# weihaoysgs/ssvio

Hardware: AMD Instinct MI355X
Metric: stereo frames/s (ORB extract + row-band match + triangulate + one local BA per frame) on 1241x376 (higher is better)
Workload: dtype u8 (front-end) + f64 (BA)

## Files before the change

### include/ssx_test_hooks.h

```cpp
#ifndef SSX_TEST_HOOKS_H
#define SSX_TEST_HOOKS_H
#include "ssx.h"

#ifdef __cplusplus
extern "C" {
#endif

SSX_API int32_t ssx_ba_window_selftest(uint32_t seed, int32_t steps);

SSX_API int64_t ssx_debug_kernel_dynamic_lds(const char* kernel);
SSX_API void ssx_debug_set_dense_slabs(int32_t mode);

SSX_API void ssx_debug_set_trial_finish(int32_t mode);

SSX_API double ssx_ba_debug_prepare_seconds(const ssx_ba_problem* prob, int32_t reps);

SSX_API int32_t ssx_ba_debug_upload_format(const ssx_ba_problem* prob);

SSX_API uint64_t ssx_ba_debug_prepare_digest(const ssx_ba_problem* prob, int32_t threads);

typedef struct ssx_orb_plan_info {
  int32_t status, n_buffers;
  uint64_t digest[3];
  uint64_t arena_bytes, buf_off[32], buf_bytes[32];
  int32_t nlevels, out_cap;
  int32_t lvl_rows[8], lvl_cols[8], feat[8], lvl_cell0[9], gauss_tile0[9];
  char error[256];
} ssx_orb_plan_info;
SSX_API ssx_status ssx_orb_debug_plan(int32_t rows, int32_t cols, int32_t images, const ssx_orb_params* prm, int32_t has_mask,
                                      int32_t detect_only, int32_t unchecked, ssx_orb_plan_info* out);


// ... 46 lines not shown
```

### ssvio_amd/csrc/ba.hip

```cpp
#include <algorithm>
#include <atomic>
#include <chrono>
#include <cmath>
#include <limits>
#include <map>
#include <condition_variable>
#include <functional>
#include <mutex>
#include <numeric>
#include <thread>
#include <unordered_map>
#include <vector>

#include <cstring>
#include <rocprim/device/device_radix_sort.hpp>
#include <rocprim/device/device_run_length_encode.hpp>
#include <rocprim/device/device_scan.hpp>

#include "ctx.hpp"
#include "se3.hpp"
#include "../../include/ssx_test_hooks.h"

int ssx_comm_allreduce_f64(void* user, double* buf_dev, size_t count, void* stream);

// ... 11 lines not shown
#ifndef SSX_LIN_VA
#define SSX_LIN_VA 14
#endif
#ifndef SSX_LS_WGS
#define SSX_LS_WGS 3
#endif
constexpr int CH_E = SSX_CHUNK_E;
constexpr int PW = CH_E + 2;
constexpr int CH_L = SSX_CHUNK_L;
constexpr int PL = CH_L + 1;
constexpr int SSX_BA_SMALL_P = 16;
constexpr int UPPER6 = 21;
constexpr int TOUCH_WORDS = (SSX_BA_SMALL_P * (SSX_BA_SMALL_P + 1) / 2 + SSX_BA_SMALL_P + 31) / 32;
constexpr int BSEG_PARTS = 4;
constexpr int BSEG_MIN = 8;
constexpr int MAX_PAIRS = CH_E * (SSX_BA_SMALL_P + 1) / 2 + 8;

template <class T>
struct GPtr {
  T* p;
#if defined(__HIP_DEVICE_COMPILE__)
  using G = __attribute__((address_space(1))) T*;
#else
  using G = T*;
#endif
  __host__ __device__ __forceinline__ GPtr& operator=(T* q) { p = q; return *this; }
  __host__ __device__ __forceinline__ operator G() const { return (G)p; }
  __host__ __device__ __forceinline__ G get() const { return (G)p; }
};
#if defined(__HIP_DEVICE_COMPILE__)
// ... 22 lines not shown
  GPtr<const uint8_t> e_cam;
  GPtr<const uint8_t> e_dup;
  GPtr<const double> e_uv;
  GPtr<const int8_t> blk_pa;
  GPtr<const int8_t> blk_pb;
  GPtr<const int4> ch_desc;
  GPtr<const int4> e_rec;
  GPtr<const int4> l_rec;
  GPtr<const uint16_t> pptr;
  GPtr<uint8_t> pair_a;
  GPtr<uint8_t> pair_b;
  GPtr<int> pair_ptr;
  GPtr<int4> bseg;
  GPtr<int> bseg_ptr;
  int bseg_cap;
  int dev_prep;
  int E_raw;
  GPtr<const int> r_edge_pose;
  GPtr<const int> r_edge_point;
  GPtr<const double> r_edge_uv;
  GPtr<const uint8_t> r_edge_cam;
  GPtr<const uint8_t> r_slot8;
  int no_err;
  int raw_fmt;
  GPtr<const int> lm_compact;
  GPtr<const int> pose_rank;
  GPtr<int> perm;
  GPtr<int> lm_chunk;
  GPtr<double> c2_out;
  Cam K;
// ... 486 lines not shown
{
  if (threadIdx.x == 0 && blockIdx.x == 0) d.scal[SC_LAMBDA] = lambda;
}

constexpr int LIST_MAX_BLK = SSX_BA_SMALL_P * (SSX_BA_SMALL_P + 1) / 2;
__device__ __forceinline__ void k_build_lists_body(const BaDev& d, const int c)
{
  __shared__ uint8_t sEdgeOf[CH_L][SSX_BA_SMALL_P];
  __shared__ int8_t sLead[CH];
  __shared__ int sCnt[2][LIST_MAX_BLK];
  __shared__ int sBp[LIST_MAX_BLK + 1];
  __shared__ int sLen[LIST_MAX_BLK], sK[LIST_MAX_BLK];
  __shared__ uint8_t sSorted[LIST_MAX_BLK];
  __shared__ int sMaxLen, sWaveTot[4], sWaveMax[4];
  __shared__ int sPosR[LIST_MAX_BLK + 1];
  __shared__ int sKr[LIST_MAX_BLK];
  const int t = threadIdx.x, lane = t & 63, wave = t >> 6;
  const int4 cd = d.ch_desc[c];
  const int e0 = cd.x, lm0 = cd.z, nl = cd.w;
  const int nP = d.nP, nBlk = d.nBlk;
  const unsigned long long lt_mask = (1ull << lane) - 1ull;
  if (t < cd.y) {
    const int4 er = d.e_rec[e0 + t];
    sLead[t] = (er.y >= 0 && !(er.w & 2)) ? (int8_t)er.y : (int8_t)-1;
  }
  int4 lr = make_int4(0, 0, 0, 1);
  if (t < nl) lr = d.l_rec[lm0 + t];
  __syncthreads();
  uint32_t mask = 0;
  if (t < nl && !lr.w)
// ... 44 lines not shown
    }
  }
  if (t < TOUCH_WORDS) {
    unsigned int m = 0;
    for (int b = 32 * t; b < min(32 * t + 32, nBlk + nP); ++b) {
      const bool on = b < nBlk ? (sBp[b + 1] > sBp[b]) : (d.pptr[(size_t)c * (nP + 1) + (b - nBlk) + 1] > d.pptr[(size_t)c * (nP + 1) + (b - nBlk)]);
      m |= (on || d.dense_slabs) ? 1u << (b & 31) : 0u;
    }
    d.touch[(size_t)c * TOUCH_WORDS + t] = m;
  }
  const int seg = max(BSEG_MIN, (sMaxLen + BSEG_PARTS - 1) / BSEG_PARTS);
  if (t < nBlk) {
    const int n = sBp[t + 1] - sBp[t], k = (n == 0 && !d.dense_slabs) ? 0 : max(1, (n + seg - 1) / seg);
    sK[t] = k;
    sLen[t] = k ? (n + k - 1) / k : 0;
  }
  __syncthreads();
  if (t < nBlk) {
    const int len = sLen[t];
    int rank = 0;
    for (int b = 0; b < nBlk; ++b) { const int lb = sLen[b]; rank += (lb > len) || (lb == len && b < t); }
    sSorted[rank] = (uint8_t)t;
  }
  __syncthreads();
  if (t < nBlk) sKr[t] = sK[sSorted[t]];
  __syncthreads();
  if (t == 0) {
    int pos = 0;
    for (int r = 0; r < nBlk; ++r) {
      const int k = sKr[r];
      if ((pos & 3) + k > 4) pos = (pos + 3) & ~3;
      sPosR[r] = pos;
      pos += k;
    }
    sPosR[nBlk] = pos;
    d.bseg_ptr[2 * c] = c * d.bseg_cap;
    d.bseg_ptr[2 * c + 1] = pos;
  }
  __syncthreads();
  if (t < nBlk) {
    int4* out = d.bseg + (size_t)c * d.bseg_cap;
    const int b = sSorted[t], n = sBp[b + 1] - sBp[b], k = sK[b], len = sLen[b], p0 = sPosR[t];
    for (int i = 0; i < k; ++i) out[p0 + i] = make_int4(b, sBp[b] + min(n, i * len), sBp[b] + min(n, (i + 1) * len), i | (k << 4));
    for (int q = p0 + k; q < sPosR[t + 1]; ++q) out[q] = make_int4(-1, 0, 0, 1 << 4);
  }
}
__global__ __launch_bounds__(CH) void k_build_lists(BaDev d) { k_build_lists_body(d, blockIdx.x); }
__global__ __launch_bounds__(CH) void k_build_lists_b(const BaDev* __restrict__ dv)
{
  const BaDev& d = dv[blockIdx.y];
  if ((int)blockIdx.x >= d.nCh || d.bseg_cap == 0) return;
  k_build_lists_body(d, blockIdx.x);
}

#define SSX_AS1(T) const __attribute__((address_space(1))) T*
__device__ __forceinline__ int raw_pose(const BaDev& d, int e)
{
  return (d.raw_fmt & 1) ? (int)((SSX_AS1(uint8_t))d.r_edge_pose.get())[e] : d.r_edge_pose[e];
}
// ... 263 lines not shown
        const double y2 = (Wm[a * 3 + 2] - y0 * l20 - y1 * l21) * i22;
        sY[(a * 3) * PW + t] = y0; sY[(a * 3 + 1) * PW + t] = y1; sY[(a * 3 + 2) * PW + t] = y2;
        z[a] = y0 * g0 + y1 * g1 + y2 * g2;
      }
    } else {
#pragma unroll
      for (int k = 0; k < 18; ++k) sY[k * PW + t] = 0.0;
    }
  }
  __syncthreads();

  const int nS = d.nBlk * 36;
  for (int base = 0; base < n_items; base += CH) {
    const int4 ir = item_rec;
    if (base + CH < n_items) item_rec = base + CH + t < n_items ? d.bseg[it0 + ((base + CH + t) >> 2)] : make_int4(-1, 0, 0, 1 << 4);
    const int blk = ir.x, qr = (t >> 1) & 1, qc = t & 1;
    const int q0 = ir.y, q1 = ir.z, part = ir.w & 15, parts = ir.w >> 4;
    double acc[3][3];
#pragma unroll
    for (int i = 0; i < 3; ++i)
#pragma unroll
      for (int j = 0; j < 3; ++j) acc[i][j] = 0.0;
    const double* bdp = sY + (qr * 9) * PW;
    const double* wp = sY + (qc * 9) * PW;
#pragma unroll 2
    for (int q = q0; q < q1; ++q) {
      const int ab = sPab[q];
      const int ea = ab & 0xFF, eb = ab >> 8;
      double bd[3][3], w[3][3];
#pragma unroll
      for (int i = 0; i < 3; ++i)
#pragma unroll
        for (int m = 0; m < 3; ++m) { bd[i][m] = bdp[(i * 3 + m) * PW + ea]; w[i][m] = wp[(i * 3 + m) * PW + eb]; }
#pragma unroll
      for (int i = 0; i < 3; ++i)
#pragma unroll
        for (int j = 0; j < 3; ++j) acc[i][j] = fma(bd[i][2], w[j][2], fma(bd[i][1], w[j][1], fma(bd[i][0], w[j][0], acc[i][j])));
    }
    if (__any(parts > 1)) {
#pragma unroll
      for (int i = 0; i < 3; ++i)
#pragma unroll
        for (int j = 0; j < 3; ++j) {
          const double v1 = dpp_f64<0x104>(acc[i][j]), v2 = dpp_f64<0x108>(acc[i][j]), v3 = dpp_f64<0x10C>(acc[i][j]);
          if (part == 0) {
            if (parts > 1) acc[i][j] += v1;
            if (parts > 2) acc[i][j] += v2;
            if (parts > 3) acc[i][j] += v3;
          }
        }
    }
    if (blk >= 0 && part == 0) {
#pragma unroll
      for (int i = 0; i < 3; ++i)
#pragma unroll
        for (int j = 0; j < 3; ++j) slab[blk * 36 + (3 * qr + i) * 6 + 3 * qc + j] = acc[i][j];
    }
  }
  __syncthreads();
  if (t < ne) {
#pragma unroll
    for (int a = 0; a < 6; ++a) sY[a * PW + zpos] = z[a];
  }
  __syncthreads();
  for (int base = 0; base < nP * 6 * 4; base += CH) {
    const int item = base + t;
    const bool on = item < nP * 6 * 4;
    const int idx = on ? item >> 2 : 0, part = item & 3;
    const int p = idx / 6, a = idx - p * 6;
    double acc = 0.0;
    const int s0 = on ? sPptr[p] : 0, s1 = on ? sPptr[p + 1] : 0;
// ... 421 lines not shown
#include "ba_band.inc"
#include "ba_bcr.inc"

}

namespace {
std::atomic<int> g_dense_slabs{-1};
std::atomic<int> g_trial_finish{1};
inline int dense_slabs_mode()
{
  int m = g_dense_slabs.load(std::memory_order_relaxed);
  if (m < 0) {
    m = getenv("SSX_BA_DENSE_SLABS") ? 1 : 0;
    g_dense_slabs.store(m, std::memory_order_relaxed);
  }
  return m;
}
struct HostPrep {
  int P, L, E, nP, nLm, nCh, nBlk;
  int E_raw = 0;
  int raw_fmt = 0;
  bool big = false;
  bool dev_lists = false;
  bool dev_prep = false;
  int band_w = -1;
  std::vector<int> pose_free, lm_id, lm_ptr, ch_lm;
  std::vector<uint8_t> lm_fixed, slot8;
  std::vector<int> lm_compact;
  std::vector<int> pose_rank;
  std::vector<int> ch_desc;
// ... 128 lines not shown
  DevBuf tiles;
  HostBuf tiles_h;
  DevBuf pairs_a, pairs_b, pairs_c;
  HostBuf pairs_h;
  HostPrep prep1;
  std::vector<HostPrep> preps;
  ParPool pool;
  DevBuf recs;
  HostBuf recs_h;
  DevBuf raw_d;
  HostBuf raw_h;
  struct RawEarly { bool valid = false; const void* key = nullptr; int E = 0; size_t o_pose = 0, o_point = 0, o_uv = 0, o_cam = 0; } raw_early;
  DevBuf win_stage_d;
  HostBuf win_stage_h;
  hipEvent_t ev_turn = nullptr;
};

static void ssx_ba_workspace_free(BaWorkspace* w)
{
  if (!w) return;
  g_turns.forget(w);
  if (w->ev_turn) (void)hipEventDestroy(w->ev_turn);
  w->arena.release();
  w->stage.release();
  w->scal.release();
  w->tiles.release();
  w->tiles_h.release();
  w->pairs_a.release(); w->pairs_b.release(); w->pairs_c.release(); w->pairs_h.release();
  w->win_stage_d.release(); w->win_stage_h.release();
  w->recs.release(); w->recs_h.release();
// ... 718 lines not shown
  eat_v(h.touch, (ref && !h.big) ? all : 0);
  eat_v(h.pe_edge, all); eat_v(h.sblk_pa, all); eat_v(h.sblk_pb, all); eat_v(h.spair_ptr, all);
  BandPlan bands[2];
  if (h.big) { plan_band(h.nP, 3, bands[1]); plan_bcr(h.nP, 3, bands[1].bcr); }
  const WinExt win;
  for (int v = 0; v < (h.dev_prep && !h.big ? 3 : 2); ++v)
   for (int keep_init = 0; keep_init < 2; ++keep_init)
    for (int b = 0; b < (h.big ? 2 : 1); ++b) {
      const ArenaPlan p = plan_arena(prob, h, bands[b], v == 1 ? 2 : 1, keep_init != 0, v == 2 ? &win : nullptr, h.big && h.dev_prep);
      for (const Span* s = p.spans_begin(); s != p.spans_end(); ++s) eat(&s->off, sizeof(size_t));
      eat(&p.in_bytes, sizeof(size_t)); eat(&p.total, sizeof(size_t));
    }
  return d;
}

int32_t ssx_ba_debug_upload_format(const ssx_ba_problem* prob)
{
  if (!prob) return -1;
  ssx_ctx dummy;
  static thread_local HostPrep h;
  if (prepare(&dummy, prob, h) != SSX_OK) return -1;
  return h.raw_fmt;
}
#endif

}

#include "ba_window.inc"
#include "pg.inc"
```

### ssvio_amd/csrc/ba_batch.inc

```

struct ssx_ba_batch {
  ssx_ctx* ctx = nullptr;
  int device = 0;
  int n = 0;
  ssx_ba_options opt;
  DevBuf arena_own; HostBuf stage_own, scal_own;
  DevBuf* arena = nullptr; HostBuf* stage = nullptr; HostBuf* scal = nullptr;
  std::vector<BaDev> devs;
  std::vector<std::vector<int>> perm;
  std::vector<int> P, L, E, E_raw;
  std::vector<WinExt*> exts;
  const ssx_ba_problem* probs = nullptr;
  std::vector<size_t> out_off;
  size_t out_total = 0, a_out = 0, a_gather = 0, a_head = 0, in_total = 0, o_dv = 0, o_ctrl = 0, o_ooff = 0;
  int max_ch = 1, max_rl = 1, max_rs = 1, total_ch = 0, min_ch = 0;
  bool any_solve64 = false, any_solve80 = false, any_solve = false, with_err = false, fresh = false;
  int threads = 1;
  int groups = 0;
};

namespace {

int batch_groups(int n)
{
// ... 65 lines not shown
    BigDev bd; BandDev bnd;
    fill_blob(plans[w], &probs[w], preps[w], no_band, hst + in_off[w]);
    wire_arena(plans[w], dev_base + B->a_head + in_off[w], dev_base + a_rest + rest_off[w], &probs[w], opt.huber_delta, opt.chi2_th, 1, 0,
               exts ? exts[w] : nullptr, nullptr, nullptr, nullptr, B->devs[w], bd, bnd);
    B->devs[w].store_w = opt.jac_mode == SSX_JAC_NUMERIC_G2O ? 1 : 0;
    B->devs[w].no_err = with_err ? 0 : 1;
    if (with_err) B->perm[w] = preps[w].perm;
  });
  if (q + 1 < Q) {
    const size_t b0 = in_off[q0], b1 = in_off[q1];
    if (b1 > b0) SSX_HIP_TRY(ctx, hipMemcpyAsync(dev_base + B->a_head + b0, hst + b0, b1 - b0, hipMemcpyHostToDevice, ctx->stream));
  }
  }
  const size_t up0 = Q > 1 ? in_off[(int)((long long)n * (Q - 1) / Q)] : 0;
  memcpy(hst + in_total + B->o_dv, B->devs.data(), sizeof(BaDev) * n);
  memset(hst + in_total + B->o_ctrl, 0, sizeof(int) * 3 * n);
  memcpy(hst + in_total + B->o_ooff, B->out_off.data(), sizeof(size_t) * n);
  for (int w = 0; w < n; ++w) {
    const BaDev& d = B->devs[w];
    B->max_ch = std::max(B->max_ch, d.nCh);
    B->min_ch = w == 0 ? d.nCh : std::min(B->min_ch, d.nCh);
    B->total_ch += d.nCh;
    B->max_rl = std::max(B->max_rl, (d.nP * 27 + 63) / 64);
    B->max_rs = std::max(B->max_rs, (d.nBlk * 36 + d.nP * 6 + 63) / 64);
    if (6 * d.nP <= NB) B->any_solve64 = true; else if (6 * d.nP <= 80) B->any_solve80 = true; else B->any_solve = true;
  }
  const double t_fill = ms_since(t_begin);
  SSX_HIP_TRY(ctx, hipMemcpyAsync(dev_base + B->a_head + up0, hst + up0, head_bytes - up0, hipMemcpyHostToDevice, ctx->stream));
  double t_up = 0.0;
  if (timing) { (void)hipStreamSynchronize(ctx->stream); t_up = ms_since(t_begin); }
// ... 252 lines not shown
```

### ssvio_amd/csrc/ba_marshal.inc

```

void make_chunks(HostPrep& h)
{
  h.ch_lm.clear();
  h.ch_lm.push_back(0);
  int acc_e = 0, acc_l = 0;
  for (int lc = 0; lc < h.nLm; ++lc) {
    const int k = h.lm_ptr[lc + 1] - h.lm_ptr[lc];
    if (acc_e + k > CH_E || acc_l + 1 > CH_L) {
      h.ch_lm.push_back(lc);
      acc_e = 0; acc_l = 0;
    }
    acc_e += k; acc_l += 1;
  }
  if (h.nLm > 0) h.ch_lm.push_back(h.nLm);
  h.nCh = (int)h.ch_lm.size() - 1;
  if (h.nCh < 0) h.nCh = 0;
}

struct WinExt {
  const int* r_edge_pose = nullptr; const int* r_edge_point = nullptr; const double* r_edge_uv = nullptr; const uint8_t* r_edge_cam = nullptr;
  double* pose[2] = {nullptr, nullptr}; double* point[2] = {nullptr, nullptr};
  int cur = 0;
  const int* pose_order = nullptr; int n_pose_order = 0;
  const int* lm_order = nullptr; int n_lm_order = 0;
// ... 234 lines not shown
    }
  }
}

void ref_pose_major(HostPrep& h)
{
  const int nP = h.nP, E = h.E;
  h.pe_ptr.assign(nP + 1, 0);
  for (int s = 0; s < E; ++s) { const int pf = h.pose_free[h.e_pose[s]]; if (pf >= 0) h.pe_ptr[pf + 1]++; }
  for (int p = 0; p < nP; ++p) h.pe_ptr[p + 1] += h.pe_ptr[p];
  h.pe_edge.assign(std::max(h.pe_ptr[nP], 1), 0);
  std::vector<int> fill(h.pe_ptr.begin(), h.pe_ptr.end() - 1);
  for (int s = 0; s < E; ++s) { const int pf = h.pose_free[h.e_pose[s]]; if (pf >= 0) h.pe_edge[fill[pf]++] = s; }
}

void ref_chunk_lists(HostPrep& h, bool build_lists)
{
  h.dev_lists = !build_lists;
  const int nP = h.nP, nBlk = h.nBlk;
  h.pptr.assign((size_t)h.nCh * (nP + 1) + 1, 0);
  h.pair_ptr.assign((size_t)h.nCh * (nBlk + 1) + 1, 0);
  h.pair_a.clear(); h.pair_b.clear();
  h.bseg.clear(); h.bseg_ptr.assign(2 * (size_t)h.nCh + 2, 0);
  h.touch.assign(TOUCH_WORDS * (size_t)(h.nCh + 1), 0u);
  std::vector<int> blk_of((size_t)std::max(nP, 1) * std::max(nP, 1), -1);
  for (int b = 0; b < nBlk; ++b) blk_of[(size_t)h.blk_pa[b] * nP + h.blk_pb[b]] = b;
  std::vector<int> pc(nP + 1), bc(nBlk + 1);
  std::vector<uint32_t>& tmp_pairs = h.tmp_pairs;
  std::vector<std::pair<int, int>>& order = h.tmp_order;
  h.bseg.reserve(4 * ((size_t)h.nCh * (nBlk + 8)));
  for (int c = 0; c < h.nCh; ++c) {
    const int lm0 = h.ch_lm[c], lm1 = h.ch_lm[c + 1];
    const int e0 = h.lm_ptr[lm0], e1 = h.lm_ptr[lm1];
    std::fill(pc.begin(), pc.end(), 0);
    for (int s = e0; s < e1; ++s) { const int pf = h.pose_free[h.e_pose[s]]; if (pf >= 0) pc[pf + 1]++; }
    for (int p = 0; p < nP; ++p) pc[p + 1] += pc[p];
    uint16_t* pp = &h.pptr[(size_t)c * (nP + 1)];
    for (int p = 0; p <= nP; ++p) pp[p] = (uint16_t)pc[p];
    int tail = pc[nP];
    for (int s = e0; s < e1; ++s) {
      const int pf = h.pose_free[h.e_pose[s]];
      const int pos = pf >= 0 ? pc[pf]++ : tail++;
      h.e_rec[4 * (size_t)s + 3] = (h.e_rec[4 * (size_t)s + 3] & 0xFFFF) | (pos << 16);
    }
    if (h.dev_lists) continue;
// ... 36 lines not shown
      const int seg = std::max(BSEG_MIN, (maxlen + BSEG_PARTS - 1) / BSEG_PARTS);
      const bool dense = dense_slabs_mode() != 0;
      unsigned int* tm = &h.touch[(size_t)c * TOUCH_WORDS];
      for (int b = 0; b < nBlk + nP; ++b) {
        const bool on = b < nBlk ? (bp[b + 1] > bp[b]) : (pp[b - nBlk + 1] > pp[b - nBlk]);
        if (on || dense) tm[b >> 5] |= 1u << (b & 31);
      }
      order.clear();
      for (int b = 0; b < nBlk; ++b) {
        const int n = bp[b + 1] - bp[b], k = (n == 0 && !dense) ? 0 : std::max(1, (n + seg - 1) / seg);
        order.push_back({k ? -((n + k - 1) / k) : 0, b});
      }
      std::stable_sort(order.begin(), order.end());
      h.bseg_ptr[2 * c] = (int)(h.bseg.size() / 4);
      int pos = 0;
      for (const auto& ob : order) {
        const int b = ob.second, n = bp[b + 1] - bp[b], k = (n == 0 && !dense) ? 0 : std::max(1, (n + seg - 1) / seg), len = k ? (n + k - 1) / k : 0;
        while ((pos & 3) + k > 4) { h.bseg.push_back(-1); h.bseg.push_back(0); h.bseg.push_back(0); h.bseg.push_back(1 << 4); ++pos; }
        for (int i = 0; i < k; ++i) {
          const int q0 = bp[b] - base + std::min(n, i * len), q1 = bp[b] - base + std::min(n, (i + 1) * len);
          h.bseg.push_back(b); h.bseg.push_back(q0); h.bseg.push_back(q1); h.bseg.push_back(i | (k << 4));
          ++pos;
        }
      }
      h.bseg_ptr[2 * c + 1] = (int)(h.bseg.size() / 4) - h.bseg_ptr[2 * c];
    }
  }
}

ssx_status prepare(ssx_ctx* ctx, const ssx_ba_problem* pr, HostPrep& h, bool allow_dev_prep = true, const WinExt* ext = nullptr)
{
  const bool dead_ok = ext != nullptr;
  SSX_TRY(prep_free_poses(ctx, pr, h, ext));
  const int L = h.L, E = h.E_raw;
  static const bool host_prep_env = getenv("SSX_BA_HOST_PREP") != nullptr;
  static const bool host_lists_env = getenv("SSX_BA_HOST_LISTS") != nullptr;
  h.big = h.nP > SSX_BA_SMALL_P;
  h.dev_prep = allow_dev_prep && !host_prep_env && !host_lists_env;
// ... 81 lines not shown
{
  ArenaPlan p{};
  const int P = p.P = h.P, L = p.L = h.L, E = p.E = h.E, nP = p.nP = h.nP, nLm = p.nLm = h.nLm, nCh = p.nCh = h.nCh, nBlk = p.nBlk = h.nBlk;
  const int E_raw = p.E_raw = h.E_raw, n = p.n = 6 * nP;
  const bool big = p.big = h.big, rz = p.on_dev = on_dev;
  const bool dev_prep = p.dev_prep = h.dev_prep && !big, dev_lists = p.dev_lists = h.dev_lists && !big;
  const bool host_recs = p.host_recs = !dev_prep && !rz, host_lists = !dev_lists;
  const bool big_up = big && !rz;
  const bool lm_up = (big || dev_prep) && !rz;
  p.ext = ext != nullptr;
  const bool raw_in = p.raw_in = dev_prep && !ext;
  p.cam_in = raw_in && pr->edge_cam != nullptr;
  p.have_rank = dev_prep && !h.pose_rank.empty();
  p.keep_init = keep_init && !ext;
  const bool band = p.band = big && bp.w > 0, bcr = p.bcr = band && bp.bcr.on;
  p.bseg_cap = dev_lists ? 2 * nBlk * BSEG_PARTS + 16 : 0;
  p.lin_stride = big ? 2 : nP * 27 + 2;
  const int n_pad = p.n_pad = big ? ((n + NB - 1) / NB) * NB : 0;
  const size_t nBlkS = h.sblk_pa.size();
  p.nBlkS = (int)nBlkS;
  const int raw_fmt = p.raw_fmt = raw_in ? h.raw_fmt : 0;
  const size_t I = sizeof(int), D = sizeof(double);
  Layout lay;
  auto blob = [&](bool on, size_t nbytes, size_t pad = 0, bool filled = true) { return Span{lay.take(on ? nbytes + pad : 0), on && filled ? nbytes : 0}; };
  auto scratch = [&](size_t nbytes) { return Span{lay.take(nbytes), 0}; };
  p.pose_free = blob(!rz, I * P);
  p.lm_fixed = blob(lm_up, nLm); p.lm_id = blob(lm_up, I * nLm); p.lm_ptr = blob(lm_up, I * (nLm + 1));
  p.ch_lm = blob(big_up, I * (nCh + 1));
  p.e_pose = blob(big_up, I * E); p.e_lmc = blob(big_up, I * E); p.e_cam = blob(big_up, E);
  if (host_recs) { p.e_dup = blob(true, E); p.e_uv = blob(true, D * 2 * E); }
  p.ch_desc = blob(!rz, I * 4 * (size_t)nCh, I * 4);
// ... 87 lines not shown
  put(p.pe_ptr, h.pe_ptr.data()); put(p.pe_edge, h.pe_edge.data());
  put(p.sblk_pa, h.sblk_pa.data()); put(p.sblk_pb, h.sblk_pb.data()); put(p.spair_ptr, h.spair_ptr.data());
  put(p.seg_p0, bp.seg_p0.data()); put(p.seg_m, bp.seg_m.data());
  put(p.bcr_p0, bp.bcr.p0.data()); put(p.bcr_elim, bp.bcr.elim.data());
  put(p.pose0, pr->poses); put(p.point0, pr->points);
}

void wire_arena(const ArenaPlan& p, char* base_in, char* base_rest, const ssx_ba_problem* pr, double huber_delta, double chi2_th, int world, int rank,
                const WinExt* ext, const BaDev* recs, const int* pe_ptr_dev, const int* pe_edge_dev, BaDev& d, BigDev& bd, BandDev& bnd)
{
  auto at = [&](const Span& s) -> char* { return s.off < p.in_bytes ? base_in + s.off : base_rest + (s.off - p.in_bytes); };
  auto at_if = [&](bool on, const Span& s) -> char* { return on ? at(s) : nullptr; };
  d.P = p.P; d.L = p.L; d.E = p.E; d.nP = p.nP; d.nLm = p.nLm; d.nCh = p.nCh; d.nBlk = p.nBlk; d.world = world; d.rank = rank;
  d.big = p.big ? 1 : 0; d.lin_stride = p.lin_stride;
  d.dense_slabs = dense_slabs_mode();
  d.touch = (unsigned int*)at(p.touch);
  d.store_w = 1;
  d.pose_free = (const int*)at(p.pose_free); d.ch_lm = (const int*)at(p.ch_lm);
  d.lm_fixed = (const uint8_t*)at(p.lm_fixed); d.lm_id = (const int*)at(p.lm_id); d.lm_ptr = (const int*)at(p.lm_ptr);
  d.e_pose = (const int*)at(p.e_pose); d.e_lmc = (const int*)at(p.e_lmc); d.e_cam = (const uint8_t*)at(p.e_cam);
  d.e_dup = (const uint8_t*)at(p.e_dup); d.e_uv = (const double*)at(p.e_uv);
  d.ch_desc = (const int4*)at(p.ch_desc); d.e_rec = (const int4*)at(p.e_rec); d.l_rec = (const int4*)at(p.l_rec);
  d.blk_pa = (const int8_t*)at(p.blk_pa); d.blk_pb = (const int8_t*)at(p.blk_pb); d.pptr = (const uint16_t*)at(p.pptr);
  d.pair_a = (uint8_t*)at(p.pair_a); d.pair_b = (uint8_t*)at(p.pair_b); d.pair_ptr = (int*)at(p.pair_ptr);
  d.bseg = (int4*)at(p.bseg); d.bseg_ptr = (int*)at(p.bseg_ptr);
  d.bseg_cap = p.bseg_cap; d.dev_prep = p.dev_prep ? 1 : 0; d.E_raw = p.E_raw; d.raw_fmt = p.raw_fmt;
  d.no_err = 0;
  if (p.ext) {
    d.r_edge_pose = ext->r_edge_pose; d.r_edge_point = ext->r_edge_point; d.r_edge_uv = ext->r_edge_uv; d.r_edge_cam = ext->r_edge_cam;
    d.pose[0] = ext->pose[0]; d.pose[1] = ext->pose[1]; d.point[0] = ext->point[0]; d.point[1] = ext->point[1];
// ... 45 lines not shown
ssx_status upload(ssx_ctx* ctx, const ssx_ba_problem* pr, const HostPrep& h, double huber_delta, double chi2_th, int world, int rank, BaDev& d, BigDev& bd,
                  const BandPlan& bp, BandDev& bnd, const WinExt* ext = nullptr, const BaDev* recs = nullptr, const int* pe_ptr_dev = nullptr, const int* pe_edge_dev = nullptr)
{
  BaWorkspace* ws = ba_workspace(ctx);
  const ArenaPlan p = plan_arena(pr, h, bp, world, false, ext, recs != nullptr);
  if (p.ext && !p.dev_prep) { ctx->set_error("ssx_ba: a window needs the device-side marshalling (<= %d free keyframes, no SSX_BA_HOST_PREP)", SSX_BA_SMALL_P); return SSX_ERR_UNSUPPORTED; }
  SSX_HIP_TRY(ctx, hipSetDevice(ctx->device));
  SSX_HIP_TRY(ctx, ws->arena.reserve(p.total));
  SSX_HIP_TRY(ctx, ws->stage.reserve(std::max(p.in_bytes, sizeof(double) * (7 * (size_t)p.P + 3 * (size_t)p.L + 2 * (size_t)p.E + (size_t)p.E_raw))));
  SSX_HIP_TRY(ctx, ws->scal.reserve(sizeof(double) * (SC_N + 3 * SSX_BA_MAX_STATS)));
  char* hs = ws->stage.as<char>();
  char* base = ws->arena.as<char>();
  fill_blob(p, pr, h, bp, hs);
  SSX_HIP_TRY(ctx, hipMemcpyAsync(base, hs, p.in_bytes, hipMemcpyHostToDevice, ctx->stream));
  wire_arena(p, base, base + p.in_bytes, pr, huber_delta, chi2_th, world, rank, ext, recs, pe_ptr_dev, pe_edge_dev, d, bd, bnd);
  if (p.pose0.n) SSX_HIP_TRY(ctx, hipMemcpyAsync(d.pose[1], d.pose[0], p.pose0.n, hipMemcpyDeviceToDevice, ctx->stream));
  if (p.point0.n) SSX_HIP_TRY(ctx, hipMemcpyAsync(d.point[1], d.point[0], p.point0.n, hipMemcpyDeviceToDevice, ctx->stream));
  if (p.nCh > 0 && (p.dev_lists || p.dev_prep)) {
    if (p.dev_prep) {
      hipLaunchKernelGGL(k_prep_scatter, dim3((p.E_raw + CH - 1) / CH), dim3(CH), 0, ctx->stream, d);
      hipLaunchKernelGGL(k_prep_chunk, dim3(p.nCh), dim3(CH), 0, ctx->stream, d);
    } else {
      hipLaunchKernelGGL(k_build_lists, dim3(p.nCh), dim3(CH), 0, ctx->stream, d);
    }
    SSX_HIP_TRY(ctx, hipGetLastError());
  }
  return SSX_OK;
}

ssx_status raw_upload_early(ssx_ctx* ctx, const ssx_ba_problem* pr)
// ... 219 lines not shown
```

Before: 17860.

## Exploit symmetry of diagonal Schur blocks with triangle and half-block work items

Diagonal pose-pose Schur blocks (pa==pb) are now split into new work-item kinds. Upper-triangle 3x3 diagonal sub-blocks are computed once and mirrored (BSEG_TRI), and the single off-diagonal 3x3 quarter is computed and stored transposed (BSEG_DIAG01). This drops the redundant lower-quarter computation on diagonal blocks. In exchange it adds more item-list layout, padding and a larger bseg capacity. Debug hooks expose the item lists, and an env var restores the old full-block path.

```diff
diff --git a/include/ssx_test_hooks.h b/include/ssx_test_hooks.h
--- a/include/ssx_test_hooks.h
+++ b/include/ssx_test_hooks.h
@@ -16,6 +16,13 @@
 SSX_API double ssx_ba_debug_prepare_seconds(const ssx_ba_problem* prob, int32_t reps);
 
 SSX_API int32_t ssx_ba_debug_upload_format(const ssx_ba_problem* prob);
+
+typedef struct ssx_ba_schur_items {
+  int32_t window, chunk, items, padding, tri_groups, diag_items, offdiag_items, diag_full_items, diag_parts_hist[4];
+} ssx_ba_schur_items;
+SSX_API ssx_status ssx_ba_debug_schur_items(ssx_ctx* ctx, int32_t cap, ssx_ba_schur_items* out, int32_t* n_out);
+SSX_API int32_t ssx_ba_debug_host_items(const ssx_ba_problem* prob, int32_t diag_full, int32_t dense, int32_t cap_items, int32_t* items, int32_t cap_chunks,
+                                        int32_t* item_ptr, int32_t cap_pair_ptr, int32_t* pair_ptr, int8_t* blk_pa, int8_t* blk_pb, int32_t* dims);
 
 SSX_API uint64_t ssx_ba_debug_prepare_digest(const ssx_ba_problem* prob, int32_t threads);
 
diff --git a/ssvio_amd/csrc/ba.hip b/ssvio_amd/csrc/ba.hip
--- a/ssvio_amd/csrc/ba.hip
+++ b/ssvio_amd/csrc/ba.hip
@@ -49,6 +49,10 @@
 constexpr int TOUCH_WORDS = (SSX_BA_SMALL_P * (SSX_BA_SMALL_P + 1) / 2 + SSX_BA_SMALL_P + 31) / 32;
 constexpr int BSEG_PARTS = 4;
 constexpr int BSEG_MIN = 8;
+constexpr int BSEG_QUARTERS = 0;
+constexpr int BSEG_TRI = 1;
+constexpr int BSEG_DIAG01 = 2;
+__host__ __device__ constexpr int bseg_capacity(int nBlk, int nP) { return 2 * nBlk * BSEG_PARTS + 3 * nP + 32; }
 constexpr int MAX_PAIRS = CH_E * (SSX_BA_SMALL_P + 1) / 2 + 8;
 
 template <class T>
@@ -101,6 +105,7 @@
   GPtr<int4> bseg;
   GPtr<int> bseg_ptr;
   int bseg_cap;
+  int diag_full;
   int dev_prep;
   int E_raw;
   GPtr<const int> r_edge_pose;
@@ -617,6 +622,8 @@
   __shared__ uint8_t sSorted[LIST_MAX_BLK];
   __shared__ int sMaxLen, sWaveTot[4], sWaveMax[4];
   __shared__ int sPosR[LIST_MAX_BLK + 1];
+  __shared__ int sPosT[LIST_MAX_BLK + 1];
+  __shared__ uint8_t sDiag[LIST_MAX_BLK];
   __shared__ int sKr[LIST_MAX_BLK];
   const int t = threadIdx.x, lane = t & 63, wave = t >> 6;
   const int4 cd = d.ch_desc[c];
@@ -691,6 +698,7 @@
     const int n = sBp[t + 1] - sBp[t], k = (n == 0 && !d.dense_slabs) ? 0 : max(1, (n + seg - 1) / seg);
     sK[t] = k;
     sLen[t] = k ? (n + k - 1) / k : 0;
+    sDiag[t] = (!d.diag_full && d.blk_pa[t] == d.blk_pb[t]) ? 1 : 0;
   }
   __syncthreads();
   if (t < nBlk) {
@@ -700,15 +708,23 @@
     sSorted[rank] = (uint8_t)t;
   }
   __syncthreads();
-  if (t < nBlk) sKr[t] = sK[sSorted[t]];
+  if (t < nBlk) { const int b = sSorted[t]; sKr[t] = sK[b] | (sDiag[b] << 8); }
   __syncthreads();
   if (t == 0) {
     int pos = 0;
     for (int r = 0; r < nBlk; ++r) {
-      const int k = sKr[r];
-      if ((pos & 3) + k > 4) pos = (pos + 3) & ~3;
+      const int g = (sKr[r] >> 8) ? ((sKr[r] & 0xFF) + 1) >> 1 : 0;
+      if ((pos & 3) + g > 4) pos = (pos + 3) & ~3;
+      sPosT[r] = pos;
+      pos += g;
+    }
+    pos = (pos + 15) & ~15;
+    sPosT[nBlk] = pos;
+    for (int r = 0; r < nBlk; ++r) {
+      const int k = sKr[r] & 0xFF, g = (sKr[r] >> 8) ? min(k, 1) : k;
+      if ((pos & 3) + g > 4) pos = (pos + 3) & ~3;
       sPosR[r] = pos;
-      pos += k;
+      pos += g;
     }
     sPosR[nBlk] = pos;
     d.bseg_ptr[2 * c] = c * d.bseg_cap;
@@ -717,9 +733,18 @@
   __syncthreads();
   if (t < nBlk) {
     int4* out = d.bseg + (size_t)c * d.bseg_cap;
-    const int b = sSorted[t], n = sBp[b + 1] - sBp[b], k = sK[b], len = sLen[b], p0 = sPosR[t];
-    for (int i = 0; i < k; ++i) out[p0 + i] = make_int4(b, sBp[b] + min(n, i * len), sBp[b] + min(n, (i + 1) * len), i | (k << 4));
-    for (int q = p0 + k; q < sPosR[t + 1]; ++q) out[q] = make_int4(-1, 0, 0, 1 << 4);
+    const int b = sSorted[t], n = sBp[b + 1] - sBp[b], k = sK[b], len = sLen[b], p0 = sPosR[t], t0 = sPosT[t];
+    int gT = 0, gR = k;
+    if (sDiag[b]) {
+      gT = (k + 1) >> 1; gR = min(k, 1);
+      for (int j = 0; j < gT; ++j)
+        out[t0 + j] = make_int4(b, sBp[b] + min(n, 2 * j * len), sBp[b] + min(n, (2 * j + (2 * j + 1 < k ? 2 : 1)) * len), (2 * j) | (k << 4) | (BSEG_TRI << 8) | (len << 16));
+      if (k) out[p0] = make_int4(b, sBp[b], sBp[b] + n, (k << 4) | (BSEG_DIAG01 << 8) | (len << 16));
+    } else {
+      for (int i = 0; i < k; ++i) out[p0 + i] = make_int4(b, sBp[b] + min(n, i * len), sBp[b] + min(n, (i + 1) * len), i | (k << 4));
+    }
+    for (int q = t0 + gT; q < sPosT[t + 1]; ++q) out[q] = make_int4(-1, 0, 0, (1 << 4) | (BSEG_TRI << 8));
+    for (int q = p0 + gR; q < sPosR[t + 1]; ++q) out[q] = make_int4(-1, 0, 0, 1 << 4);
   }
 }
 __global__ __launch_bounds__(CH) void k_build_lists(BaDev d) { k_build_lists_body(d, blockIdx.x); }
@@ -1013,8 +1038,54 @@
   for (int base = 0; base < n_items; base += CH) {
     const int4 ir = item_rec;
     if (base + CH < n_items) item_rec = base + CH + t < n_items ? d.bseg[it0 + ((base + CH + t) >> 2)] : make_int4(-1, 0, 0, 1 << 4);
-    const int blk = ir.x, qr = (t >> 1) & 1, qc = t & 1;
-    const int q0 = ir.y, q1 = ir.z, part = ir.w & 15, parts = ir.w >> 4;
+    const int blk = ir.x, kind = (ir.w >> 8) & 3, parts = (ir.w >> 4) & 15, len = (ir.w >> 16) & 0xFF;
+    if (__any(kind == BSEG_TRI)) {
+      const int tri = t & 1, sub = (t >> 1) & 1;
+      const int mid = min(ir.z, ir.y + len);
+      const int q0 = sub ? mid : ir.y, q1 = sub ? ir.z : mid, part = (ir.w & 15) + sub;
+      double acc[6] = {0.0, 0.0, 0.0, 0.0, 0.0, 0.0};
+      const double* yp = sY + (tri * 9) * PW;
+#pragma unroll 2
+      for (int q = q0; q < q1; ++q) {
+        const int ea = sPab[q] & 0xFF;
+        double y[3][3];
+#pragma unroll
+        for (int i = 0; i < 3; ++i)
+#pragma unroll
+          for (int m = 0; m < 3; ++m) y[i][m] = yp[(i * 3 + m) * PW + ea];
+        int k = 0;
+#pragma unroll
+        for (int i = 0; i < 3; ++i)
+#pragma unroll
+          for (int j = i; j < 3; ++j, ++k) acc[k] = fma(y[i][2], y[j][2], fma(y[i][1], y[j][1], fma(y[i][0], y[j][0], acc[k])));
+      }
+      if (__any(parts > 1)) {
+#pragma unroll
+        for (int k = 0; k < 6; ++k) {
+          const double v1 = dpp_f64<0x102>(acc[k]), v2 = dpp_f64<0x104>(acc[k]), v3 = dpp_f64<0x106>(acc[k]);
+          if (part == 0) {
+            if (parts > 1) acc[k] += v1;
+            if (parts > 2) acc[k] += v2;
+            if (parts > 3) acc[k] += v3;
+          }
+        }
+      }
+      if (blk >= 0 && part == 0) {
+        int k = 0;
+#pragma unroll
+        for (int i = 0; i < 3; ++i)
+#pragma unroll
+          for (int j = i; j < 3; ++j, ++k) {
+            slab[blk * 36 + (3 * tri + i) * 6 + 3 * tri + j] = acc[k];
+            if (j > i) slab[blk * 36 + (3 * tri + j) * 6 + 3 * tri + i] = acc[k];
+          }
+      }
+      continue;
+    }
+    const bool dg = kind == BSEG_DIAG01;
+    const int qr = dg ? 0 : (t >> 1) & 1, qc = dg ? 1 : t & 1;
+    const int part = dg ? t & 3 : ir.w & 15;
+    const int q0 = dg ? min(ir.z, ir.y + part * len) : ir.y, q1 = dg ? min(ir.z, ir.y + (part + 1) * len) : ir.z;
     double acc[3][3];
 #pragma unroll
     for (int i = 0; i < 3; ++i)
@@ -1041,11 +1112,12 @@
       for (int i = 0; i < 3; ++i)
 #pragma unroll
         for (int j = 0; j < 3; ++j) {
-          const double v1 = dpp_f64<0x104>(acc[i][j]), v2 = dpp_f64<0x108>(acc[i][j]), v3 = dpp_f64<0x10C>(acc[i][j]);
+          const double u1 = dpp_f64<0x104>(acc[i][j]), u2 = dpp_f64<0x108>(acc[i][j]), u3 = dpp_f64<0x10C>(acc[i][j]);
+          const double d1 = dpp_f64<0x101>(acc[i][j]), d2 = dpp_f64<0x102>(acc[i][j]), d3 = dpp_f64<0x103>(acc[i][j]);
           if (part == 0) {
-            if (parts > 1) acc[i][j] += v1;
-            if (parts > 2) acc[i][j] += v2;
-            if (parts > 3) acc[i][j] += v3;
+            if (parts > 1) acc[i][j] += dg ? d1 : u1;
+            if (parts > 2) acc[i][j] += dg ? d2 : u2;
+            if (parts > 3) acc[i][j] += dg ? d3 : u3;
           }
         }
     }
@@ -1053,7 +1125,10 @@
 #pragma unroll
       for (int i = 0; i < 3; ++i)
 #pragma unroll
-        for (int j = 0; j < 3; ++j) slab[blk * 36 + (3 * qr + i) * 6 + 3 * qc + j] = acc[i][j];
+        for (int j = 0; j < 3; ++j) {
+          slab[blk * 36 + (3 * qr + i) * 6 + 3 * qc + j] = acc[i][j];
+          if (dg) slab[blk * 36 + (3 * qc + j) * 6 + 3 * qr + i] = acc[i][j];
+        }
     }
   }
   __syncthreads();
@@ -1505,6 +1580,11 @@
     m = getenv("SSX_BA_DENSE_SLABS") ? 1 : 0;
     g_dense_slabs.store(m, std::memory_order_relaxed);
   }
+  return m;
+}
+inline int diag_full_mode()
+{
+  static const int m = getenv("SSX_BA_DIAG_FULL") ? 1 : 0;
   return m;
 }
 struct HostPrep {
@@ -1663,6 +1743,7 @@
   DevBuf win_stage_d;
   HostBuf win_stage_h;
   hipEvent_t ev_turn = nullptr;
+  std::vector<BaDev> last_devs;
 };
 
 static void ssx_ba_workspace_free(BaWorkspace* w)
@@ -2411,6 +2492,66 @@
   return d;
 }
 
+ssx_status ssx_ba_debug_schur_items(ssx_ctx* ctx, int32_t cap, ssx_ba_schur_items* out, int32_t* n_out)
+{
+  if (!ctx || !n_out || (cap > 0 && !out)) return SSX_ERR_INVALID_ARG;
+  BaWorkspace* ws = ba_workspace(ctx);
+  *n_out = 0;
+  SSX_HIP_TRY(ctx, hipSetDevice(ctx->device));
+  SSX_HIP_TRY(ctx, hipStreamSynchronize(ctx->stream));
+  std::vector<int> ptr, items;
+  std::vector<int8_t> pa, pb;
+  for (size_t w = 0; w < ws->last_devs.size(); ++w) {
+    const BaDev& d = ws->last_devs[w];
+    if (d.big || d.nCh <= 0 || d.nBlk <= 0) continue;
+    ptr.resize(2 * (size_t)d.nCh); pa.resize(d.nBlk); pb.resize(d.nBlk);
+    SSX_HIP_TRY(ctx, hipMemcpy(ptr.data(), d.bseg_ptr.p, sizeof(int) * ptr.size(), hipMemcpyDeviceToHost));
+    SSX_HIP_TRY(ctx, hipMemcpy(pa.data(), d.blk_pa.p, d.nBlk, hipMemcpyDeviceToHost));
+    SSX_HIP_TRY(ctx, hipMemcpy(pb.data(), d.blk_pb.p, d.nBlk, hipMemcpyDeviceToHost));
+    for (int c = 0; c < d.nCh; ++c) {
+      const int n = ptr[2 * c + 1];
+      if (n < 0 || (d.bseg_cap && n > d.bseg_cap)) { ctx->set_error("ssx_ba_debug_schur_items: chunk %d holds %d items, %d reserved", c, n, d.bseg_cap); return SSX_ERR_CAPACITY; }
+      items.resize(4 * (size_t)std::max(n, 1));
+      if (n) SSX_HIP_TRY(ctx, hipMemcpy(items.data(), d.bseg.p + ptr[2 * c], sizeof(int) * 4 * (size_t)n, hipMemcpyDeviceToHost));
+      ssx_ba_schur_items r{};
+      r.window = (int32_t)w; r.chunk = c; r.items = n;
+      for (int i = 0; i < n; ++i) {
+        const int blk = items[4 * i], wd = items[4 * i + 3], kind = (wd >> 8) & 3, k = (wd >> 4) & 15;
+        if (blk < 0) { r.padding++; continue; }
+        const bool diag = pa[blk] == pb[blk];
+        if (kind == BSEG_TRI) r.tri_groups++;
+        else if (kind == BSEG_DIAG01) { r.diag_items++; if (k >= 1 && k <= 4) r.diag_parts_hist[k - 1]++; }
+        else if (kind == BSEG_QUARTERS && diag) { r.diag_full_items++; if ((wd & 15) == 0 && k >= 1 && k <= 4) r.diag_parts_hist[k - 1]++; }
+        else r.offdiag_items++;
+      }
+      if (*n_out < cap) out[*n_out] = r;
+      ++*n_out;
+    }
+  }
+  return SSX_OK;
+}
+
+int32_t ssx_ba_debug_host_items(const ssx_ba_problem* prob, int32_t diag_full, int32_t dense, int32_t cap_items, int32_t* items, int32_t cap_chunks,
+                                int32_t* item_ptr, int32_t cap_pair_ptr, int32_t* pair_ptr, int8_t* blk_pa, int8_t* blk_pb, int32_t* dims)
+{
+  if (!prob || !items || !item_ptr || !pair_ptr || !blk_pa || !blk_pb || !dims) return -1;
+  ssx_ctx dummy;
+  static thread_local HostPrep h;
+  if (prepare(&dummy, prob, h, false) != SSX_OK || h.big) return -1;
+  const int keep = g_dense_slabs.load();
+  if (dense >= 0) g_dense_slabs.store(dense ? 1 : 0);
+  ref_chunk_lists(h, true, diag_full);
+  g_dense_slabs.store(keep);
+  const int n = (int)(h.bseg.size() / 4);
+  dims[0] = h.nCh; dims[1] = h.nBlk; dims[2] = h.nP;
+  if (n > cap_items || h.nCh > cap_chunks || (size_t)h.nCh * (h.nBlk + 1) > (size_t)cap_pair_ptr || h.nBlk > LIST_MAX_BLK) return -1;
+  memcpy(items, h.bseg.data(), sizeof(int) * 4 * (size_t)n);
+  memcpy(item_ptr, h.bseg_ptr.data(), sizeof(int) * 2 * (size_t)h.nCh);
+  memcpy(pair_ptr, h.pair_ptr.data(), sizeof(int) * (size_t)h.nCh * (h.nBlk + 1));
+  memcpy(blk_pa, h.blk_pa.data(), h.nBlk); memcpy(blk_pb, h.blk_pb.data(), h.nBlk);
+  return n;
+}
+
 int32_t ssx_ba_debug_upload_format(const ssx_ba_problem* prob)
 {
   if (!prob) return -1;
diff --git a/ssvio_amd/csrc/ba_batch.inc b/ssvio_amd/csrc/ba_batch.inc
--- a/ssvio_amd/csrc/ba_batch.inc
+++ b/ssvio_amd/csrc/ba_batch.inc
@@ -103,6 +103,7 @@
   }
   const size_t up0 = Q > 1 ? in_off[(int)((long long)n * (Q - 1) / Q)] : 0;
   memcpy(hst + in_total + B->o_dv, B->devs.data(), sizeof(BaDev) * n);
+  ws->last_devs = B->devs;
   memset(hst + in_total + B->o_ctrl, 0, sizeof(int) * 3 * n);
   memcpy(hst + in_total + B->o_ooff, B->out_off.data(), sizeof(size_t) * n);
   for (int w = 0; w < n; ++w) {
diff --git a/ssvio_amd/csrc/ba_marshal.inc b/ssvio_amd/csrc/ba_marshal.inc
--- a/ssvio_amd/csrc/ba_marshal.inc
+++ b/ssvio_amd/csrc/ba_marshal.inc
@@ -272,8 +272,9 @@
   for (int s = 0; s < E; ++s) { const int pf = h.pose_free[h.e_pose[s]]; if (pf >= 0) h.pe_edge[fill[pf]++] = s; }
 }
 
-void ref_chunk_lists(HostPrep& h, bool build_lists)
-{
+void ref_chunk_lists(HostPrep& h, bool build_lists, int diag_full = -1)
+{
+  if (diag_full < 0) diag_full = diag_full_mode();
   h.dev_lists = !build_lists;
   const int nP = h.nP, nBlk = h.nBlk;
   h.pptr.assign((size_t)h.nCh * (nP + 1) + 1, 0);
@@ -286,7 +287,7 @@
   std::vector<int> pc(nP + 1), bc(nBlk + 1);
   std::vector<uint32_t>& tmp_pairs = h.tmp_pairs;
   std::vector<std::pair<int, int>>& order = h.tmp_order;
-  h.bseg.reserve(4 * ((size_t)h.nCh * (nBlk + 8)));
+  h.bseg.reserve(4 * ((size_t)h.nCh * (nBlk + nP + 24)));
   for (int c = 0; c < h.nCh; ++c) {
     const int lm0 = h.ch_lm[c], lm1 = h.ch_lm[c + 1];
     const int e0 = h.lm_ptr[lm0], e1 = h.lm_ptr[lm1];
@@ -353,14 +354,28 @@
       std::stable_sort(order.begin(), order.end());
       h.bseg_ptr[2 * c] = (int)(h.bseg.size() / 4);
       int pos = 0;
+      auto item = [&](int b, int q0, int q1, int w) { h.bseg.push_back(b); h.bseg.push_back(q0); h.bseg.push_back(q1); h.bseg.push_back(w); ++pos; };
+      auto parts_of = [&](int b, int& n, int& k, int& len) { n = bp[b + 1] - bp[b]; k = (n == 0 && !dense) ? 0 : std::max(1, (n + seg - 1) / seg); len = k ? (n + k - 1) / k : 0; };
       for (const auto& ob : order) {
-        const int b = ob.second, n = bp[b + 1] - bp[b], k = (n == 0 && !dense) ? 0 : std::max(1, (n + seg - 1) / seg), len = k ? (n + k - 1) / k : 0;
-        while ((pos & 3) + k > 4) { h.bseg.push_back(-1); h.bseg.push_back(0); h.bseg.push_back(0); h.bseg.push_back(1 << 4); ++pos; }
-        for (int i = 0; i < k; ++i) {
-          const int q0 = bp[b] - base + std::min(n, i * len), q1 = bp[b] - base + std::min(n, (i + 1) * len);
-          h.bseg.push_back(b); h.bseg.push_back(q0); h.bseg.push_back(q1); h.bseg.push_back(i | (k << 4));
-          ++pos;
-        }
+        const int b = ob.second;
+        int n, k, len;
+        parts_of(b, n, k, len);
+        if (diag_full || h.blk_pa[b] != h.blk_pb[b]) continue;
+        const int g = (k + 1) / 2;
+        while ((pos & 3) + g > 4) item(-1, 0, 0, (1 << 4) | (BSEG_TRI << 8));
+        for (int j = 0; j < g; ++j)
+          item(b, bp[b] - base + std::min(n, 2 * j * len), bp[b] - base + std::min(n, (2 * j + (2 * j + 1 < k ? 2 : 1)) * len), (2 * j) | (k << 4) | (BSEG_TRI << 8) | (len << 16));
+      }
+      while (pos & 15) item(-1, 0, 0, (1 << 4) | (BSEG_TRI << 8));
+      for (const auto& ob : order) {
+        const int b = ob.second;
+        int n, k, len;
+        parts_of(b, n, k, len);
+        const bool dg = !diag_full && h.blk_pa[b] == h.blk_pb[b];
+        const int g = dg ? std::min(k, 1) : k;
+        while ((pos & 3) + g > 4) item(-1, 0, 0, 1 << 4);
+        if (dg) { if (k) item(b, bp[b] - base, bp[b] - base + n, (k << 4) | (BSEG_DIAG01 << 8) | (len << 16)); continue; }
+        for (int i = 0; i < k; ++i) item(b, bp[b] - base + std::min(n, i * len), bp[b] - base + std::min(n, (i + 1) * len), i | (k << 4));
       }
       h.bseg_ptr[2 * c + 1] = (int)(h.bseg.size() / 4) - h.bseg_ptr[2 * c];
     }
@@ -472,7 +487,7 @@
   p.have_rank = dev_prep && !h.pose_rank.empty();
   p.keep_init = keep_init && !ext;
   const bool band = p.band = big && bp.w > 0, bcr = p.bcr = band && bp.bcr.on;
-  p.bseg_cap = dev_lists ? 2 * nBlk * BSEG_PARTS + 16 : 0;
+  p.bseg_cap = dev_lists ? bseg_capacity(nBlk, nP) : 0;
   p.lin_stride = big ? 2 : nP * 27 + 2;
   const int n_pad = p.n_pad = big ? ((n + NB - 1) / NB) * NB : 0;
   const size_t nBlkS = h.sblk_pa.size();
@@ -590,6 +605,7 @@
   d.P = p.P; d.L = p.L; d.E = p.E; d.nP = p.nP; d.nLm = p.nLm; d.nCh = p.nCh; d.nBlk = p.nBlk; d.world = world; d.rank = rank;
   d.big = p.big ? 1 : 0; d.lin_stride = p.lin_stride;
   d.dense_slabs = dense_slabs_mode();
+  d.diag_full = diag_full_mode();
   d.touch = (unsigned int*)at(p.touch);
   d.store_w = 1;
   d.pose_free = (const int*)at(p.pose_free); d.ch_lm = (const int*)at(p.ch_lm);
@@ -665,6 +681,7 @@
   fill_blob(p, pr, h, bp, hs);
   SSX_HIP_TRY(ctx, hipMemcpyAsync(base, hs, p.in_bytes, hipMemcpyHostToDevice, ctx->stream));
   wire_arena(p, base, base + p.in_bytes, pr, huber_delta, chi2_th, world, rank, ext, recs, pe_ptr_dev, pe_edge_dev, d, bd, bnd);
+  ws->last_devs.assign(1, d);
   if (p.pose0.n) SSX_HIP_TRY(ctx, hipMemcpyAsync(d.pose[1], d.pose[0], p.pose0.n, hipMemcpyDeviceToDevice, ctx->stream));
   if (p.point0.n) SSX_HIP_TRY(ctx, hipMemcpyAsync(d.point[1], d.point[0], p.point0.n, hipMemcpyDeviceToDevice, ctx->stream));
   if (p.nCh > 0 && (p.dev_lists || p.dev_prep)) {
```

Result: slower. 17560 (-1.6%).
